# ChenAnno/FashionERN_AAAI2024

Hardware: AMD Instinct MI355X
Metric: composed queries/sec (higher is better)
Workload: dtype f32; 1 GPU; FashionIQ ViT-B/16 composed queries: 64-query batch per GPU vs 46k-image fused gallery (BASELINE.json configs[1]); clip=ViT-B-16, query_batch_per_gpu=64, gallery_rows=46000, gallery_dtype=f32, feature_dim=512, top_k=50, batches_in_flight=4, hw_queues=4, parallelism=dp1 queries

## Files before the change

### fashionern_aaai2024_amd/_lib.py

```python
from __future__ import annotations

import ctypes as C
import os

from . import build as _build

c_void_p, c_int, c_i64, c_float = C.c_void_p, C.c_int, C.c_int64, C.c_float

os.environ.setdefault("GPU_MAX_HW_QUEUES", "8")


class ClipConfigC(C.Structure):
    _fields_ = [(n, c_int) for n in (
        "embed_dim", "image_size", "patch_size", "v_width", "v_layers", "v_heads", "v_mlp",
        "context_length", "vocab_size", "t_width", "t_heads", "t_layers", "t_mlp", "v_arch")] + [
        ("r_layers", c_int * 4), ("r_width", c_int), ("r_heads", c_int)]


class ProfStats(C.Structure):
    _fields_ = [("gemm_ms", C.c_double), ("gemm_flops", C.c_double), ("gemm_launches", c_i64),
                ("attn_ms", C.c_double), ("attn_flops", C.c_double), ("attn_launches", c_i64),
                ("topk_ms", C.c_double), ("topk_launches", c_i64),
                ("sweep_ms", C.c_double), ("sweep_bytes", C.c_double), ("sweep_launches", c_i64),
                ("gemm_fp8_ms", C.c_double), ("gemm_fp8_flops", C.c_double), ("gemm_fp8_launches", c_i64),
# ... 73 lines not shown
    "fern_set_precision": (c_int, [c_void_p, c_int]),
    "fern_get_precision": (c_int, [c_void_p]),
    "fern_gemm_bf16": (c_int, [c_void_p, c_void_p, c_i64, c_void_p, c_i64, c_void_p, c_void_p, c_void_p, c_i64,
                               c_int, c_int, c_int, c_int, c_int, c_void_p]),
    "fern_quantize_rows_fp8": (c_int, [c_void_p, c_void_p, c_int, c_i64, c_void_p, c_i64, c_void_p, c_i64, c_int, c_void_p]),
    "fern_gemm_fp8": (c_int, [c_void_p, c_void_p, c_i64, c_void_p, c_void_p, c_i64, c_void_p, c_void_p, c_void_p, c_void_p, c_i64,
                              c_int, c_int, c_int, c_int, c_int, c_void_p]),
    "fern_quantize_mx8": (c_int, [c_void_p, c_void_p, c_int, c_i64, c_void_p, c_i64, c_void_p, c_i64, c_i64, c_int, c_void_p]),
    "fern_gemm_mx8": (c_int, [c_void_p, c_void_p, c_i64, c_void_p, c_i64, c_void_p, c_i64, c_void_p, c_i64, c_void_p, c_void_p, c_void_p, c_i64,
                              c_int, c_int, c_int, c_int, c_int, c_void_p]),
    "fern_gemm_mx8_quant": (c_int, [c_void_p, c_void_p, c_i64, c_void_p, c_i64, c_void_p, c_i64, c_void_p, c_i64, c_void_p, c_void_p, c_i64,
                                    c_void_p, c_i64, c_int, c_int, c_int, c_int, c_void_p]),
    "fern_layernorm": (c_int, [c_void_p, c_void_p, c_void_p, c_void_p, c_void_p, c_void_p, c_i64, c_int, c_float, c_void_p]),
    "fern_attention": (c_int, [c_void_p, c_void_p, c_i64, c_void_p, c_i64, c_void_p, c_i64, c_void_p, c_i64,
                               c_int, c_int, c_int, c_int, c_int, c_int, c_float, c_void_p]),
    "fern_attention_bf16": (c_int, [c_void_p, c_void_p, c_i64, c_void_p, c_i64, c_void_p, c_i64, c_void_p, c_i64,
                                    c_int, c_int, c_int, c_int, c_int, c_int, c_float, c_void_p]),
    "fern_layernorm_q": (c_int, [c_void_p, c_void_p, c_int, c_i64, c_void_p, c_void_p, c_int, c_void_p, c_i64, c_void_p, c_i64, c_i64,
                                 c_int, c_float, c_void_p]),
    "fern_attention_mx8": (c_int, [c_void_p, c_void_p, c_i64, c_void_p, c_i64, c_void_p, c_i64, c_void_p, c_i64, c_void_p, c_i64,
                                   c_int, c_int, c_int, c_int, c_int, c_int, c_float, c_void_p]),
    "fern_im2col_q": (c_int, [c_void_p, c_void_p, c_int, c_int, c_int, c_int, c_void_p, c_void_p, c_i64, c_void_p]),
    "fern_prof_enable": (c_int, [c_void_p, c_int]),
    "fern_prof_collect": (c_int, [c_void_p, C.POINTER(ProfStats)]),
    "fern_tuner_export": (c_i64, [C.c_char_p, c_i64]),
    "fern_tuner_import": (c_int, [C.c_char_p]),
    "fern_tuner_set_concurrency": (c_int, [c_int]),
    "fern_tuner_force_config": (c_int, [C.c_char_p, c_int]),
    "fern_ws_generation": (C.c_uint64, [c_void_p]),
}
# ... 34 lines not shown
```

### fashionern_aaai2024_amd/csrc/api_blocks.hip

```cpp
#include "ctx.h"

using namespace fern;
using namespace fern::api;

extern "C" int fern_resample_u8_horizontal(fern_ctx* c, const uint8_t* src, int64_t src_ld, int x0, int y0, int rows, uint8_t* dst, int ow,
                                           const int32_t* bounds, const int32_t* coeffs, int ksize, void* stream) {
    if (!c || !src || !dst || !bounds || !coeffs || rows < 0 || ow < 0 || ksize < 1) return fail(FERN_ERR_ARG, "fern_resample_u8_horizontal: bad argument");
    HIP_TRY(hipSetDevice(c->device));
    HIP_TRY(launch_resample_h(src, src_ld, x0, y0, rows, dst, ow, bounds, coeffs, ksize, (hipStream_t)stream));
    return FERN_OK;
}
extern "C" int fern_resample_u8_vertical(fern_ctx* c, const uint8_t* src, int64_t src_ld, int x0, int y0, int cols, uint8_t* dst, int oh,
                                         const int32_t* bounds, const int32_t* coeffs, int ksize, void* stream) {
    if (!c || !src || !dst || !bounds || !coeffs || cols < 0 || oh < 0 || ksize < 1) return fail(FERN_ERR_ARG, "fern_resample_u8_vertical: bad argument");
    HIP_TRY(hipSetDevice(c->device));
    HIP_TRY(launch_resample_v(src, src_ld, x0, y0, cols, dst, oh, bounds, coeffs, ksize, (hipStream_t)stream));
    return FERN_OK;
}
extern "C" int fern_u8_to_normalized_chw(fern_ctx* c, const uint8_t* src, int64_t src_ld, int x0, int y0, int64_t src_image_stride, float* dst,
                                         int n, int oh, int ow, const float* host_mean, const float* host_std, void* stream) {
    if (!c || !src || !dst || !host_mean || !host_std || n < 0 || oh < 0 || ow < 0) return fail(FERN_ERR_ARG, "fern_u8_to_normalized_chw: bad argument");
    HIP_TRY(hipSetDevice(c->device));
    HIP_TRY(launch_u8_to_chw(src, src_ld, x0, y0, dst, n, src_image_stride, oh, ow, host_mean, host_std, (hipStream_t)stream));
    return FERN_OK;
// ... 142 lines not shown
                              int64_t ldo, int batch, int heads, int head_dim, int s_q, int s_k, int causal, float scale, void* stream) {
    FERN_TRY(attn_begin(c, "fern_attention", q, k, v, out, ldq, ldk, ldv, ldo, heads, head_dim));
    AttnParams a{q, k, v, out, (long)ldq, (long)ldk, (long)ldv, (long)ldo, batch, heads, head_dim, s_q, s_k, causal, scale};
    return run_attention(c, a, (hipStream_t)stream);
}

extern "C" int fern_attention_bf16(fern_ctx* c, const uint16_t* q, int64_t ldq, const uint16_t* k, int64_t ldk, const uint16_t* v, int64_t ldv,
                                   uint16_t* out, int64_t ldo, int batch, int heads, int head_dim, int s_q, int s_k, int causal, float scale,
                                   void* stream) {
    FERN_TRY(attn_begin(c, "fern_attention_bf16", q, k, v, out, ldq, ldk, ldv, ldo, heads, head_dim));
    return run_attention(c, attn_desc_b(q, ldq, k, ldk, v, ldv, out, ldo, batch, heads, head_dim, s_q, s_k, causal, scale), (hipStream_t)stream);
}

static bool misaligned16(const void* p) { return (reinterpret_cast<uintptr_t>(p) & 15) != 0; }

extern "C" int fern_layernorm_q(fern_ctx* c, const void* x, int x_is_bf16, int64_t ldx, const float* gamma, const float* beta, int out_form,
                                void* y, int64_t ldy, void* scales, int64_t scale_rows, int64_t rows, int d, float eps, void* stream) {
    if (!c) return fail(FERN_ERR_ARG, "fern_layernorm_q: ctx is NULL");
    if (rows < 0 || (out_form != FERN_QFORM_BF16 && out_form != FERN_QFORM_FP8 && out_form != FERN_QFORM_MX8))
        return fail(FERN_ERR_ARG, "fern_layernorm_q: bad argument");
    if (rows == 0) return FERN_OK;
    if (!x || !gamma || !beta || !y || (out_form != FERN_QFORM_BF16 && !scales)) return fail(FERN_ERR_ARG, "fern_layernorm_q: NULL argument");
    if (d <= 0 || d % 4 || d > 1280 || ldx < d || ldy < d || ldx % 4 || ldy % 4)
        return fail(FERN_ERR_ARG, "fern_layernorm_q: need d % 4 == 0, d <= 1280, ld % 4 == 0, ld >= d");
    if (misaligned16(x) || misaligned16(gamma) || misaligned16(beta) || misaligned16(y) || (scales && misaligned16(scales)))
        return fail(FERN_ERR_ARG, "fern_layernorm_q: pointers must be 16-byte aligned");
    if (out_form == FERN_QFORM_MX8 && (d % 128 || scale_rows < rows))
        return fail(FERN_ERR_ARG, "fern_layernorm_q: the MX form needs d % 128 == 0 and scale_rows >= rows");
    if (out_form != FERN_QFORM_MX8 && x_is_bf16) return fail(FERN_ERR_ARG, "fern_layernorm_q: bf16 rows are read by the MX form only");
    HIP_TRY(hipSetDevice(c->device));
// ... 55 lines not shown
```

### fashionern_aaai2024_amd/csrc/api_ctx.hip

```cpp
#include <cstdio>
#include <cstdlib>
#include <cstring>
#include "ctx.h"

using namespace fern;
using namespace fern::api;

static thread_local std::string g_last_error;
int fern::api::fail(int code, const std::string& msg) {
    g_last_error = msg;
    return code;
}
extern "C" int fern_abi_version(void) { return FERN_ABI_VERSION; }
extern "C" const char* fern_last_error(void) { return g_last_error.c_str(); }

namespace fern {
thread_local LaunchTimer* g_launch_timer = nullptr;
hipEvent_t launch_timer_event() {
    LaunchTimer* t = g_launch_timer;
    hipEvent_t e = nullptr;
    if (t && t->pool && !t->pool->empty()) { e = t->pool->back(); t->pool->pop_back(); }
    else (void)hipEventCreate(&e);
    return e;
}
// ... 277 lines not shown
    const hipError_t le = launch_gemm_mxbf_pair(p1, p2, s);
    HIP_TRY_PROF(le, c, slot);
    if (slot >= 0) {
        c->recs[slot].dispatches = gemm_last_dispatches();
        c->recs[slot].extra_flops = 2.0 * p2.M * (double)p2.N * p2.K;
    }
    return prof_close(c, slot, s);
}
int fern::api::run_attention(fern_ctx* c, const AttnParams& a, hipStream_t s) {
    int slot;
    FERN_TRY(prof_open(c, PROF_ATTN, 4.0 * a.batch * a.heads * (double)a.s_q * a.s_k * a.hd, s, &slot, a.batch * a.heads, a.s_q, a.hd, a.causal));
    const hipError_t le = launch_attention(a, s);
    HIP_TRY_PROF(le, c, slot);
    return prof_close(c, slot, s);
}

extern "C" int fern_set_precision(fern_ctx* c, int precision) {
    if (!c) return fail(FERN_ERR_ARG, "fern_set_precision: ctx is NULL");
    if (precision != FERN_PREC_FP32 && precision != FERN_PREC_BF16 && precision != FERN_PREC_FP8 && precision != FERN_PREC_MX8 &&
        precision != FERN_PREC_F32X3 && precision != FERN_PREC_MX8_MLP && precision != FERN_PREC_MX8_IMG)
        return fail(FERN_ERR_ARG, "fern_set_precision: unknown precision");
    const bool split = precision == FERN_PREC_F32X3;
    if (split) precision = FERN_PREC_FP32;
    auto every_layer_has = [&](const unsigned char* LinearW::*copy) {
        for (const auto* blocks : {&c->clip.vblocks, &c->clip.tblocks})
            for (const auto& b : *blocks)
                if (!(b.qkv.*copy) || !(b.out.*copy) || !(b.fc.*copy) || !(b.proj.*copy)) return false;
        return true;
    };
    if ((precision == FERN_PREC_MX8 || precision == FERN_PREC_MX8_MLP || precision == FERN_PREC_MX8_IMG) && c->clip.ready && !every_layer_has(&LinearW::wm))
// ... 49 lines not shown
```

### fashionern_aaai2024_amd/csrc/api_towers.hip

```cpp
#include <cmath>
#include "ctx.h"

using namespace fern;
using namespace fern::api;

enum Form { F32, BF16, FP8, MX };

struct Tower {
    const ClipBlockW* blocks;
    int batch, S, width, heads, mlp, causal;
    Form attn, mlpf;
    bool bf16_stream;
    float *X, *XN, *QKV, *ATT, *H;
    unsigned short* Xb;

    long R() const { return (long)batch * S; }
    void* stream() const { return Xb ? (void*)Xb : (void*)X; }
    unsigned short* XNb() const { return reinterpret_cast<unsigned short*>(XN); }
    unsigned short* QKVb() const { return reinterpret_cast<unsigned short*>(QKV); }
    unsigned short* ATTb() const { return reinterpret_cast<unsigned short*>(ATT); }
    unsigned short* Hb() const { return reinterpret_cast<unsigned short*>(H); }
    unsigned char* XN8() const { return reinterpret_cast<unsigned char*>(XN); }
    float* SA() const { return XN + ((size_t)R() * width / 4 + 63) / 64 * 64; }
    unsigned char* SM() const { return reinterpret_cast<unsigned char*>(SA()); }
// ... 129 lines not shown
    FERN_TRY(run_gemm_form(c, T.mlpf, p, s));
    FERN_TRY(prep_proj(c, T, Bk, s, &p));
    return run_gemm_form(c, T.mlpf, p, s);
}

static int clip_block_cls_only(fern_ctx* c, const Tower& V, const ClipBlockW& Bk, float* CLS , float* T0 ,
                               float* T1 , float* H , hipStream_t s) {
    const int batch = V.batch, S = V.S, width = V.width, heads = V.heads, hd = width / heads;
    const float* X = V.X;
    const unsigned short* Xb = V.Xb;
    float* QKV = V.QKV;
    LinearW kv{Bk.qkv.w + (size_t)width * width, Bk.qkv.b + width, 2 * width, width, Bk.qkv.wb + (size_t)width * width,
               Bk.qkv.w8 ? Bk.qkv.w8 + (size_t)width * width : nullptr, Bk.qkv.sw ? Bk.qkv.sw + width : nullptr,
               Bk.qkv.wm ? Bk.qkv.wm + (size_t)width * width : nullptr, Bk.qkv.swm ? Bk.qkv.swm + (size_t)width * 4 : nullptr, Bk.qkv.swm_rows};
    const Form f = c->precision == FERN_PREC_MX8_IMG ? BF16 : V.attn;
    GemmParams pk;
    FERN_TRY(ln_gemm(V, f, Bk.ln1, kv, QKV + width, 3 * width, EPI_BIAS, false, s, &pk));
    FERN_TRY(run_gemm_form(c, f, pk, s));
    if (f == F32) {
        HIP_TRY(launch_gather_rows(V.XN, width, T0, width, batch, width, 1, S, 0, nullptr, s));
    } else {
        if (Xb) HIP_TRY(launch_gather_rows_bf16(Xb, width, T1, width, batch, width, S, s));
        else HIP_TRY(launch_gather_rows(X, width, T1, width, batch, width, 1, S, 0, nullptr, s));
        HIP_TRY(launch_layernorm(T1, nullptr, Bk.ln1.g, Bk.ln1.b, T0, batch, width, width, width, 1e-5f, s));
    }
    LinearW qw{Bk.qkv.w, Bk.qkv.b, width, width};
    FERN_TRY(run_gemm(c, gemm_desc(T0, width, qw, T1, width, batch, EPI_BIAS), s));
    AttnParams a{T1, QKV + width, QKV + 2 * width, T0, (long)width, 3L * width, 3L * width, (long)width,
                 batch, heads, hd, 1, S, 0, 1.0f / std::sqrt((float)hd)};
    FERN_TRY(run_attention(c, a, s));
    if (Xb) HIP_TRY(launch_gather_rows_bf16(Xb, width, CLS, width, batch, width, S, s));
    else HIP_TRY(launch_gather_rows(X, width, CLS, width, batch, width, 1, S, 0, nullptr, s));
    GemmParams po = gemm_desc(T0, width, Bk.out, CLS, width, batch, EPI_BIAS_RESIDUAL);
    po.R = CLS;
    FERN_TRY(run_gemm(c, po, s));
    HIP_TRY(launch_layernorm(CLS, nullptr, Bk.ln2.g, Bk.ln2.b, T0, batch, width, width, width, 1e-5f, s));
    FERN_TRY(run_gemm(c, gemm_desc(T0, width, Bk.fc, H, Bk.fc.out, batch, clip_mlp_epi(c)), s));
    GemmParams p2 = gemm_desc(H, Bk.fc.out, Bk.proj, CLS, width, batch, EPI_BIAS_RESIDUAL);
    p2.R = CLS;
    const int ks = (Bk.fc.out >= 2048 && Bk.fc.out % 512 == 0 && (width & 3) == 0) ? Bk.fc.out / 512 : 1;
    if (ks > 1) {
        float* kpart;
        FERN_TRY(ws_get(c, (size_t)ks * batch * width, &kpart));
        p2.ksplit = ks; p2.kpart = kpart; p2.epi = EPI_BIAS; p2.R = nullptr;
        FERN_TRY(run_gemm(c, p2, s));
// ... 113 lines not shown
static int resnet_chunk(fern_ctx* c, const float* images, float* out, int b, hipStream_t s) {
    const ClipW& W = c->clip;
    const ResNetW& R = W.res;
    const fern_clip_config& cf = W.cfg;
    const int S = cf.image_size, s1 = S / 2, w = cf.r_width;
    size_t max_act = (size_t)b * s1 * s1 * std::max(R.stem_c, w);
    {
        int H = S / 4;
        for (const auto& B : R.blocks) {
            max_act = std::max(max_act, (size_t)b * H * H * std::max(B.cin, B.planes * 4));
            if (B.stride > 1) H /= 2;
        }
    }
    {
        const int hf = S / 32;
        max_act = std::max(max_act, (size_t)b * (hf * hf + 1) * 2 * (size_t)(w * 32));
    }
    float* buf[6];
    for (auto& p : buf) FERN_TRY(ws_get(c, max_act, &p));
    HIP_TRY(launch_stem_conv(images, R.stem1.w, R.stem1.b, buf[0], b, S, R.stem_c, s));
    FERN_TRY(conv3x3(c, buf[0], R.stem2, buf[1], b, s1, s1, R.stem_c, s));
    FERN_TRY(conv3x3(c, buf[1], R.stem3, buf[0], b, s1, s1, R.stem_c, s));
    HIP_TRY(launch_avgpool_nhwc(buf[0], buf[1], b, s1, s1, w, 2, s));
    float* X = buf[1];
    float* OUT = buf[0];
    int H = S / 4;
    for (const auto& B : R.blocks) {
        const int rows = b * H * H, Ho = H / B.stride, rows_o = b * Ho * Ho;
        float *T1 = buf[2], *T2 = buf[3], *TP = buf[4], *ID = buf[5];
        FERN_TRY(run_gemm(c, conv_desc(X, B.c1, T1, rows, EPI_BIAS_RELU), s));
        FERN_TRY(conv3x3(c, T1, B.c2, T2, b, H, H, B.planes, s));
// ... 5 lines not shown
            HIP_TRY(launch_avgpool_nhwc(X, TP, b, H, H, B.cin, B.stride, s));
            xin = TP;
        }
        const float* identity = X;
        if (B.has_down) {
            FERN_TRY(run_gemm(c, conv_desc(xin, B.down, ID, rows_o, EPI_BIAS), s));
            identity = ID;
        }
        GemmParams p3 = conv_desc(t2, B.c3, OUT, rows_o, EPI_BIAS_RESIDUAL_RELU);
        p3.R = identity;
        FERN_TRY(run_gemm(c, p3, s));
        std::swap(X, OUT);
        H = Ho;
    }
    const int HW = H * H, E = w * 32, heads = cf.r_heads, hd = E / heads;
    float *T = buf[2], *T0 = buf[3], *MEAN = buf[3] + (size_t)b * E, *KV = buf[4], *Q = buf[5], *ATT = buf[5] + (size_t)b * E;
    HIP_TRY(launch_attnpool_tokens(X, MEAN, R.pos, T, T0, b, HW, E, s));
    FERN_TRY(run_gemm(c, gemm_desc(T, E, R.kv, KV, 2 * E, b * (HW + 1), EPI_BIAS), s));
    FERN_TRY(run_gemm(c, gemm_desc(T0, E, R.q, Q, E, b, EPI_BIAS), s));
    AttnParams a{Q, KV, KV + E, ATT, (long)E, 2L * E, 2L * E, (long)E, b, heads, hd, 1, HW + 1, 0, 1.0f / std::sqrt((float)hd)};
    FERN_TRY(run_attention(c, a, s));
    return run_gemm(c, gemm_desc(ATT, E, R.cproj, out, cf.embed_dim, b, EPI_BIAS), s);
}

extern "C" int fern_vit_encode_image(fern_ctx* c, const float* images, float* out, int b, void* stream) {
    if (!c) return fail(FERN_ERR_ARG, "fern_vit_encode_image: ctx is NULL");
    if (!c->clip.ready || (c->clip.cfg.v_arch == 0 && c->clip.cfg.v_layers <= 0))
        return fail(FERN_ERR_STATE, "fern_vit_encode_image: image tower not finalised (fern_finalize_clip)");
    FERN_TRY(check_fresh(c, "fern_vit_encode_image"));
    if (b < 0 || (b && (!images || !out))) return fail(FERN_ERR_ARG, "fern_vit_encode_image: bad argument");
    HIP_TRY(hipSetDevice(c->device));
    hipStream_t s = (hipStream_t)stream;
    const fern_clip_config& cf = c->clip.cfg;
    const long img_sz = 3L * cf.image_size * cf.image_size;
    const bool resnet = cf.v_arch == 1;
    const int CH = resnet ? 128 : vit_chunk_images(cf);
// ... 123 lines not shown
```

### fashionern_aaai2024_amd/csrc/attn.hip

```cpp
#include "kernels.h"

#include <cstdlib>

namespace fern {

typedef float f32x16 __attribute__((ext_vector_type(16)));
typedef float f32x4 __attribute__((ext_vector_type(4)));
typedef short bf16x8 __attribute__((ext_vector_type(8)));
typedef short s16x4 __attribute__((ext_vector_type(4)));
typedef unsigned u32x4_t __attribute__((ext_vector_type(4)));

extern __shared__ __attribute__((aligned(16))) char attn_smem[];

struct LanePos { int l31, lh, tr_off; };
__device__ __forceinline__ LanePos lane_pos() {
    const int lane = threadIdx.x & 63, lh = lane >> 5;
    return {lane & 31, lh, ((lane & 15) >> 2) * 64 + (((lane >> 4) & 1) * 16 + (lane & 3) * 4) * 2 + lh * 4 * 64};
}

template <int HDP_>
struct F32Form {
    static constexpr int HDP = HDP_;
    static constexpr bool BF16 = false;
    static constexpr int KS = HDP + 4;
// ... 464 lines not shown
        for (int u = 0; u < UNR; ++u) {
            const int j = j0 + 4 * u;
            vv[u] = vb[(long)(j < p.s_k ? j : p.s_k - 1) * p.ldv];
        }
#pragma unroll
        for (int u = 0; u < UNR; ++u) {
            const int j = j0 + 4 * u;
            acc = __builtin_fmaf(j < p.s_k ? sc[j] : 0.0f, vv[u], acc);
        }
    }
    red[wave][lane] = acc;
    __syncthreads();
    if (wave == 0 && lane < hd)
        p.out[(long)b * p.ldo + (long)h * hd + lane] = (((red[0][lane] + red[1][lane]) + red[2][lane]) + red[3][lane]) * (1.0f / sum);
}
hipError_t launch_attention(const AttnParams& p, hipStream_t s) {
    if (p.batch <= 0 || p.heads <= 0 || p.s_q <= 0 || p.s_k <= 0 || p.s_k > ATTN_MAX_KEYS) return hipErrorInvalidValue;
    if (p.causal && p.s_q != p.s_k) return hipErrorInvalidValue;
    if (p.qb || p.kb || p.vb) {
        if (!p.qb || !p.kb || !p.vb || (!p.out_b && !p.out_q8) || (p.out_q8 && (!p.out_scales || (p.hd & 31))) || (p.hd & 7) || (p.ldq & 7) || (p.ldk & 7) || (p.ldv & 7) || (p.ldo & 3)) return hipErrorInvalidValue;
        return launch_hd<Bf16Form>(p, s);
    }
    if (p.out_b || p.out_q8) return hipErrorInvalidValue;
    if ((p.hd & 3) || (p.ldq & 3) || (p.ldk & 3) || (p.ldv & 3) || (p.ldo & 3)) return hipErrorInvalidValue;
    if (p.s_q == 1 && !p.causal && p.hd <= 64 && p.s_k <= SQ1_MAX_KEYS) {
        FERN_LAUNCH(attn_f32_single_query_kernel<25>, dim3(p.batch * p.heads), dim3(256), 0, s, p);
        return hipGetLastError();
    }
    return launch_hd<F32Form>(p, s);
}
// ... 3 lines not shown
```

### fashionern_aaai2024_amd/csrc/ctx.h

```cpp
#pragma once
#include <hip/hip_runtime.h>
#include <algorithm>
#include <cstdint>
#include <map>
#include <string>
#include <vector>
#include "../../include/fern.h"
#include "kernels.h"

namespace fern::api {
int fail(int code, const std::string& msg);

#define HIP_TRY(expr)                                                                                   \
    do {                                                                                                \
        hipError_t e_ = (expr);                                                                         \
        if (e_ != hipSuccess)                                                                           \
            return ::fern::api::fail(e_ == hipErrorInvalidValue ? FERN_ERR_ARG : FERN_ERR_HIP,          \
                        std::string(#expr) + ": " + hipGetErrorString(e_) + " (" __FILE__ ":" + std::to_string(__LINE__) + ")"); \
    } while (0)
#define FERN_TRY(expr)              \
    do {                            \
        int r_ = (expr);            \
        if (r_ != FERN_OK) return r_; \
    } while (0)
// ... 122 lines not shown
    bool on = false, done = false;
    int sweep_lo = 0, sweep_hi = 0;
    double sweep_bytes = 0;
    StageTimer(fern_ctx* ctx, hipStream_t s);
    void sweep_begin() { if (on) sweep_lo = (int)c->timer.events.size() / 2; }
    void sweep_end(double bytes) { if (on) { sweep_hi = (int)c->timer.events.size() / 2; sweep_bytes += bytes; } }
    void commit(int m, int n, int k);
    ~StageTimer();
};

int run_gemm(fern_ctx* c, const GemmParams& p, hipStream_t s, int kind = PROF_GEMM, double work = -1.0);
int run_gemm_pair(fern_ctx* c, const GemmParams& p1, const GemmParams& p2, hipStream_t s);
int run_gemm_b(fern_ctx* c, const GemmParams& p, hipStream_t s);
int run_gemm_b_pair(fern_ctx* c, const GemmParams& p1, const GemmParams& p2, hipStream_t s);
int run_attention(fern_ctx* c, const AttnParams& a, hipStream_t s);
GemmParams gemm_desc(const float* A, long lda, const LinearW& L, float* C, long ldc, int M, int epi);
GemmParams gemm_desc_b(const unsigned short* A, long lda, const LinearW& L, void* C, long ldc, int M, int epi, bool out_bf16);
GemmParams gemm_desc_f8(const unsigned char* A8, const float* sa, long lda, const LinearW& L, void* C, long ldc, int M, int epi, bool out_bf16);
GemmParams gemm_desc_mx(const unsigned char* A8, const unsigned char* sa, long srows, long lda, const LinearW& L, void* C, long ldc, int M, int epi, bool out_bf16);
int clip_mlp_epi(const fern_ctx* c);

int check_fresh(fern_ctx* c, const char* fn);
int check_token_flag(fern_ctx* c, const char* fn);
int check_live_flags(fern_ctx* c, const char* fn);

}
```

### fashionern_aaai2024_amd/csrc/kernels.h

```cpp
#pragma once
#include <hip/hip_runtime.h>
#include <stdint.h>

#include <string>

#ifdef __HIPCC__
#include <hip/hip_ext.h>
#endif
#include <vector>

namespace fern {

struct LaunchTimer {
    std::vector<hipEvent_t> events;
    std::vector<hipEvent_t>* pool;
};
extern thread_local LaunchTimer* g_launch_timer;
struct LaunchTimerPause {
    LaunchTimer* saved;
    LaunchTimerPause() : saved(g_launch_timer) { g_launch_timer = nullptr; }
    ~LaunchTimerPause() { g_launch_timer = saved; }
};
hipEvent_t launch_timer_event();
#ifdef __HIPCC__
// ... 201 lines not shown
struct AttnParams {
    const float* q; const float* k; const float* v; float* out;
    long ldq, ldk, ldv, ldo;
    int batch, heads, hd, s_q, s_k, causal;
    float scale;
    unsigned short* out_b;
    const unsigned short* qb;
    const unsigned short* kb;
    const unsigned short* vb;
    unsigned char* out_q8;
    unsigned char* out_scales;
    long out_srows;
};
constexpr int ATTN_MAX_KEYS = 4096;
hipError_t launch_attention(const AttnParams& p, hipStream_t s);

hipError_t launch_layernorm(const float* x, const float* res, const float* gamma, const float* beta, float* y,
                            long rows, int d, long ldx, long ldy, float eps, hipStream_t s);
hipError_t launch_layernorm_bf16(const float* x, const float* gamma, const float* beta, unsigned short* y, long rows, int d, long ldx,
                                 long ldy, float eps, hipStream_t s);
hipError_t launch_layernorm_fp8(const float* x, const float* gamma, const float* beta, unsigned char* y, float* scale, long rows, int d,
                                long ldx, long ldy, float eps, hipStream_t s);
hipError_t launch_quantize_rows_fp8(const unsigned short* x_bf16, const float* x_f32, long ldx, unsigned char* y, long ldy, float* scale,
                                    long rows, int d, hipStream_t s);
hipError_t launch_layernorm_mx8(const float* x, const float* gamma, const float* beta, unsigned char* y, unsigned char* scales, long srows,
                                long rows, int d, long ldx, long ldy, float eps, hipStream_t s, const unsigned short* x_bf16 = nullptr );
hipError_t launch_quantize_mx8(const unsigned short* x_bf16, const float* x_f32, long ldx, unsigned char* y, long ldy, unsigned char* scales,
                               long srows, long rows, int d, hipStream_t s);
hipError_t launch_im2col_bf16(const float* images, unsigned short* y, int b, int img, int patch, int grid, hipStream_t s);
hipError_t launch_patch_rows_f32(const float* images, float* y, int b, int img, int patch, int grid, int kp, hipStream_t s);
// ... 108 lines not shown
```

### fashionern_aaai2024_amd/engine.py

```python
from __future__ import annotations

import ctypes as C
import sys
from typing import Dict, Mapping, Optional

import numpy as np
import torch

from . import _lib
from .synth import ClipConfig

COMBINER_TARGET, COMBINER_DVR_GLOBAL, COMBINER_DVR_LOCAL, COMBINER_DVR_FINAL = 0, 1, 2, 3
SR_TARGET, SR_DVR = 0, 1
EPI_BIAS, EPI_BIAS_GELU, EPI_BIAS_RELU, EPI_BIAS_RESIDUAL = 0, 1, 2, 3
EPI_BIAS_QUICKGELU = 4
ACT_GELU, ACT_QUICK_GELU = 0, 1
PART_DVR, PART_TARGET_SR, PART_TARGET_COMBINER, PART_ALL = 1, 2, 4, 7
PREC_FP32, PREC_BF16, PREC_FP8, PREC_MX8, PREC_F32X3, PREC_MX8_MLP, PREC_MX8_IMG = 0, 1, 2, 3, 4, 5, 6
QFORM_BF16, QFORM_FP8, QFORM_MX8 = 0, 1, 2
_PREC_NAMES = {"fp32": PREC_FP32, "bf16": PREC_BF16, "fp8": PREC_FP8, "mx8": PREC_MX8, "f32x3": PREC_F32X3, "mx8mlp": PREC_MX8_MLP, "mx8img": PREC_MX8_IMG}
PATCH_NUM = 13


def _ptr(t: Optional[torch.Tensor]):
# ... 810 lines not shown
        _lib.check(self.lib.fern_layernorm(self._h, _ptr(x), _ptr(residual), _ptr(gamma), _ptr(beta), _ptr(out), rows, d,
                                           float(eps), _stream()), "fern_layernorm")
        return out

    def attention(self, q, k, v, heads: int, causal=False, scale=None) -> torch.Tensor:
        q, k, v = self._f32(q), self._f32(k), self._f32(v)
        b, sq, w = q.shape
        sk = k.shape[1]
        hd = w // heads
        out = torch.empty_like(q)
        sc = float(scale) if scale is not None else hd ** -0.5
        _lib.check(self.lib.fern_attention(self._h, _ptr(q), w, _ptr(k), w, _ptr(v), w, _ptr(out), w, b, heads, hd, sq, sk,
                                           int(bool(causal)), sc, _stream()), "fern_attention")
        return out

    def attention_bf16(self, q, k, v, heads: int, causal=False, scale=None) -> torch.Tensor:
        def b16(x):
            if x.dtype != torch.bfloat16:
                x3 = self._f32(x)
                return self.to_bf16(x3.reshape(-1, x3.shape[-1])).reshape(x3.shape)
            return x.to(self.device).contiguous()
        q, k, v = b16(q), b16(k), b16(v)
        b, sq, w = q.shape
        sk = k.shape[1]
        hd = w // heads
        out = torch.empty_like(q)
        sc = float(scale) if scale is not None else hd ** -0.5
        _lib.check(self.lib.fern_attention_bf16(self._h, _ptr(q), w, _ptr(k), w, _ptr(v), w, _ptr(out), w, b, heads, hd, sq, sk,
                                                int(bool(causal)), sc, _stream()), "fern_attention_bf16")
        return out
# ... 86 lines not shown
```

### include/fern.h

```cpp
#ifndef FERN_H
#define FERN_H

#include <stddef.h>
#include <stdint.h>

#ifdef __cplusplus
extern "C" {
#endif

#define FERN_ABI_VERSION 3

#if defined(__GNUC__)
#define FERN_API __attribute__((visibility("default")))
#else
#define FERN_API
#endif

typedef struct fern_ctx fern_ctx;

typedef enum {
    FERN_OK = 0,
    FERN_ERR_ARG = -1,
    FERN_ERR_HIP = -2,
    FERN_ERR_STATE = -3,
// ... 235 lines not shown
                  const float* scale_w, const float* bias, const float* residual, void* C, int64_t ldc, int M, int N, int K,
                  int epilogue, int out_bf16, void* stream);
FERN_API int fern_quantize_mx8(fern_ctx* ctx, const void* x, int x_is_bf16, int64_t ldx, uint8_t* y, int64_t ldy, uint8_t* scales,
                      int64_t scale_rows, int64_t rows, int d, void* stream);
FERN_API int fern_gemm_mx8(fern_ctx* ctx, const uint8_t* A, int64_t lda, const uint8_t* scales_a, int64_t scale_rows_a, const uint8_t* W,
                  int64_t ldw, const uint8_t* scales_w, int64_t scale_rows_w, const float* bias, const float* residual, void* C,
                  int64_t ldc, int M, int N, int K, int epilogue, int out_bf16, void* stream);
FERN_API int fern_gemm_mx8_quant(fern_ctx* ctx, const uint8_t* A, int64_t lda, const uint8_t* scales_a, int64_t scale_rows_a, const uint8_t* W,
                        int64_t ldw, const uint8_t* scales_w, int64_t scale_rows_w, const float* bias, uint8_t* C8, int64_t ldc,
                        uint8_t* scales_c, int64_t scale_rows_c, int M, int N, int K, int epilogue, void* stream);
FERN_API int fern_layernorm(fern_ctx* ctx, const float* x, const float* residual, const float* gamma,
                   const float* beta, float* y, int64_t rows, int d, float eps, void* stream);
FERN_API int fern_attention(fern_ctx* ctx, const float* q, int64_t ldq, const float* k, int64_t ldk, const float* v,
                   int64_t ldv, float* out, int64_t ldo, int batch, int heads, int head_dim, int s_q,
                   int s_k, int causal, float scale, void* stream);
FERN_API int fern_attention_bf16(fern_ctx* ctx, const uint16_t* q, int64_t ldq, const uint16_t* k, int64_t ldk, const uint16_t* v,
                        int64_t ldv, uint16_t* out, int64_t ldo, int batch, int heads, int head_dim, int s_q, int s_k,
                        int causal, float scale, void* stream);
FERN_API int fern_layernorm_q(fern_ctx* ctx, const void* x, int x_is_bf16, int64_t ldx, const float* gamma, const float* beta, int out_form,
                     void* y, int64_t ldy, void* scales, int64_t scale_rows, int64_t rows, int d, float eps, void* stream);
FERN_API int fern_attention_mx8(fern_ctx* ctx, const uint16_t* q, int64_t ldq, const uint16_t* k, int64_t ldk, const uint16_t* v,
                       int64_t ldv, uint8_t* out, int64_t ldo, uint8_t* scales, int64_t scale_rows, int batch, int heads,
                       int head_dim, int s_q, int s_k, int causal, float scale, void* stream);
FERN_API int fern_im2col_q(fern_ctx* ctx, const float* images, int b, int img, int patch, int out_form, void* y, void* scales,
                  int64_t scale_rows, void* stream);

FERN_API int64_t fern_tuner_export(char* buf, int64_t cap);
FERN_API int fern_tuner_import(const char* text);
FERN_API int fern_tuner_set_concurrency(int lanes);
FERN_API int fern_tuner_force_config(const char* family, int cfg);
// ... 11 lines not shown
```

Before: 2955 queries/sec.

## Fold K/V projections into single-query pooled attention to skip full KV GEMM

For single-query attention pooling (the ViT last-block CLS path in F32 and the ResNet attnpool), the kernel stops projecting every token to K and V. It folds the query through Wk into a per-head query in token space, scores the raw tokens, takes the softmax-weighted token sum, and only then applies Wv plus bias per head. This removes the large K/V GEMM over all tokens and its activation buffer, which is why the workspace sizing shrinks. The cost is three new custom kernels plus extra per-head work, and the K bias is dropped from the scores on the assumption that it is constant across keys and cancels in the softmax.

```diff
diff --git a/fashionern_aaai2024_amd/_lib.py b/fashionern_aaai2024_amd/_lib.py
--- a/fashionern_aaai2024_amd/_lib.py
+++ b/fashionern_aaai2024_amd/_lib.py
@@ -111,6 +111,8 @@
     "fern_layernorm": (c_int, [c_void_p, c_void_p, c_void_p, c_void_p, c_void_p, c_void_p, c_i64, c_int, c_float, c_void_p]),
     "fern_attention": (c_int, [c_void_p, c_void_p, c_i64, c_void_p, c_i64, c_void_p, c_i64, c_void_p, c_i64,
                                c_int, c_int, c_int, c_int, c_int, c_int, c_float, c_void_p]),
+    "fern_pooled_attention": (c_int, [c_void_p, c_void_p, c_i64, c_void_p, c_i64, c_i64, c_void_p, c_void_p, c_void_p, c_void_p, c_i64,
+                                      c_int, c_int, c_int, c_int, c_void_p]),
     "fern_attention_bf16": (c_int, [c_void_p, c_void_p, c_i64, c_void_p, c_i64, c_void_p, c_i64, c_void_p, c_i64,
                                     c_int, c_int, c_int, c_int, c_int, c_int, c_float, c_void_p]),
     "fern_layernorm_q": (c_int, [c_void_p, c_void_p, c_int, c_i64, c_void_p, c_void_p, c_int, c_void_p, c_i64, c_void_p, c_i64, c_i64,
diff --git a/fashionern_aaai2024_amd/csrc/api_blocks.hip b/fashionern_aaai2024_amd/csrc/api_blocks.hip
--- a/fashionern_aaai2024_amd/csrc/api_blocks.hip
+++ b/fashionern_aaai2024_amd/csrc/api_blocks.hip
@@ -180,6 +180,28 @@
 
 static bool misaligned16(const void* p) { return (reinterpret_cast<uintptr_t>(p) & 15) != 0; }
 
+extern "C" int fern_pooled_attention(fern_ctx* c, const float* q, int64_t ldq, const float* tokens, int64_t ldt, int64_t image_stride,
+                                     const float* wk, const float* wv, const float* bv, float* out, int64_t ldo, int batch, int heads,
+                                     int head_dim, int s, void* stream) {
+    if (!c) return fail(FERN_ERR_ARG, "fern_pooled_attention: ctx is NULL");
+    if (!q || !tokens || !wk || !wv || !bv || !out) return fail(FERN_ERR_ARG, "fern_pooled_attention: NULL argument");
+    const int64_t E = (int64_t)heads * head_dim;
+    if (batch <= 0 || heads <= 0 || head_dim <= 0 || head_dim % 4 || head_dim > 128 || E > POOLED_MAX_E || s <= 0 || s > POOLED_MAX_KEYS)
+        return fail(FERN_ERR_ARG, "fern_pooled_attention: need head_dim % 4 == 0, head_dim <= 128, heads * head_dim <= " +
+                                      std::to_string(POOLED_MAX_E) + ", 1 <= s <= " + std::to_string(POOLED_MAX_KEYS));
+    if (ldq < E || ldt < E || ldo < E || ldq % 4 || ldt % 4 || ldo % 4 || image_stride % 4 || image_stride < (int64_t)(s - 1) * ldt + E)
+        return fail(FERN_ERR_ARG, "fern_pooled_attention: need ldq, ldt, ldo >= heads * head_dim, strides % 4 == 0, image_stride >= (s - 1) * ldt + heads * head_dim");
+    if (misaligned16(q) || misaligned16(tokens) || misaligned16(wk) || misaligned16(wv) || misaligned16(bv) || misaligned16(out))
+        return fail(FERN_ERR_ARG, "fern_pooled_attention: pointers must be 16-byte aligned");
+    HIP_TRY(hipSetDevice(c->device));
+    const hipStream_t st = (hipStream_t)stream;
+    FERN_TRY(ws_begin(c, st));
+    PooledAttnParams a{q, (long)ldq, tokens, (long)ldt, (long)image_stride, wk, wv, (long)E, bv, out, (long)ldo, nullptr, nullptr,
+                       batch, heads, head_dim, s, 1.0f / std::sqrt((float)head_dim)};
+    return run_pooled_attention(c, a, st);
+}
+
+
 extern "C" int fern_layernorm_q(fern_ctx* c, const void* x, int x_is_bf16, int64_t ldx, const float* gamma, const float* beta, int out_form,
                                 void* y, int64_t ldy, void* scales, int64_t scale_rows, int64_t rows, int d, float eps, void* stream) {
     if (!c) return fail(FERN_ERR_ARG, "fern_layernorm_q: ctx is NULL");
diff --git a/fashionern_aaai2024_amd/csrc/api_ctx.hip b/fashionern_aaai2024_amd/csrc/api_ctx.hip
--- a/fashionern_aaai2024_amd/csrc/api_ctx.hip
+++ b/fashionern_aaai2024_amd/csrc/api_ctx.hip
@@ -315,6 +315,18 @@
     HIP_TRY_PROF(le, c, slot);
     return prof_close(c, slot, s);
 }
+int fern::api::run_pooled_attention(fern_ctx* c, const PooledAttnParams& p, hipStream_t s) {
+    PooledAttnParams a = p;
+    const double E = (double)a.heads * a.hd;
+    if (a.batch <= 0 || a.heads <= 0 || a.hd <= 0) return fail(FERN_ERR_ARG, "pooled attention: bad shape");
+    FERN_TRY(ws_get(c, (size_t)a.batch * a.heads * (size_t)E, &a.qt));
+    FERN_TRY(ws_get(c, (size_t)a.batch * a.heads * (size_t)E, &a.u));
+    int slot;
+    FERN_TRY(prof_open(c, PROF_ATTN, 4.0 * a.batch * E * E + 4.0 * a.batch * a.heads * (double)a.S * E, s, &slot, a.batch * a.heads, 1, (int)E, 2));
+    const hipError_t le = launch_pooled_attention(a, s);
+    HIP_TRY_PROF(le, c, slot);
+    return prof_close(c, slot, s);
+}
 
 extern "C" int fern_set_precision(fern_ctx* c, int precision) {
     if (!c) return fail(FERN_ERR_ARG, "fern_set_precision: ctx is NULL");
diff --git a/fashionern_aaai2024_amd/csrc/api_towers.hip b/fashionern_aaai2024_amd/csrc/api_towers.hip
--- a/fashionern_aaai2024_amd/csrc/api_towers.hip
+++ b/fashionern_aaai2024_amd/csrc/api_towers.hip
@@ -167,9 +167,14 @@
                Bk.qkv.w8 ? Bk.qkv.w8 + (size_t)width * width : nullptr, Bk.qkv.sw ? Bk.qkv.sw + width : nullptr,
                Bk.qkv.wm ? Bk.qkv.wm + (size_t)width * width : nullptr, Bk.qkv.swm ? Bk.qkv.swm + (size_t)width * 4 : nullptr, Bk.qkv.swm_rows};
     const Form f = c->precision == FERN_PREC_MX8_IMG ? BF16 : V.attn;
-    GemmParams pk;
-    FERN_TRY(ln_gemm(V, f, Bk.ln1, kv, QKV + width, 3 * width, EPI_BIAS, false, s, &pk));
-    FERN_TRY(run_gemm_form(c, f, pk, s));
+    const bool pooled = f == F32 && S <= POOLED_MAX_KEYS && width <= POOLED_MAX_E && hd <= 128;
+    if (pooled) {
+        HIP_TRY(launch_layernorm(X, nullptr, Bk.ln1.g, Bk.ln1.b, V.XN, V.R(), width, width, width, 1e-5f, s));
+    } else {
+        GemmParams pk;
+        FERN_TRY(ln_gemm(V, f, Bk.ln1, kv, QKV + width, 3 * width, EPI_BIAS, false, s, &pk));
+        FERN_TRY(run_gemm_form(c, f, pk, s));
+    }
     if (f == F32) {
         HIP_TRY(launch_gather_rows(V.XN, width, T0, width, batch, width, 1, S, 0, nullptr, s));
     } else {
@@ -179,9 +184,15 @@
     }
     LinearW qw{Bk.qkv.w, Bk.qkv.b, width, width};
     FERN_TRY(run_gemm(c, gemm_desc(T0, width, qw, T1, width, batch, EPI_BIAS), s));
-    AttnParams a{T1, QKV + width, QKV + 2 * width, T0, (long)width, 3L * width, 3L * width, (long)width,
-                 batch, heads, hd, 1, S, 0, 1.0f / std::sqrt((float)hd)};
-    FERN_TRY(run_attention(c, a, s));
+    if (pooled) {
+        PooledAttnParams a{T1, (long)width, V.XN, (long)width, (long)S * width, kv.w, kv.w + (size_t)width * width, (long)width, kv.b + width,
+                           T0, (long)width, nullptr, nullptr, batch, heads, hd, S, 1.0f / std::sqrt((float)hd)};
+        FERN_TRY(run_pooled_attention(c, a, s));
+    } else {
+        AttnParams a{T1, QKV + width, QKV + 2 * width, T0, (long)width, 3L * width, 3L * width, (long)width,
+                     batch, heads, hd, 1, S, 0, 1.0f / std::sqrt((float)hd)};
+        FERN_TRY(run_attention(c, a, s));
+    }
     if (Xb) HIP_TRY(launch_gather_rows_bf16(Xb, width, CLS, width, batch, width, S, s));
     else HIP_TRY(launch_gather_rows(X, width, CLS, width, batch, width, 1, S, 0, nullptr, s));
     GemmParams po = gemm_desc(T0, width, Bk.out, CLS, width, batch, EPI_BIAS_RESIDUAL);
@@ -325,7 +336,7 @@
     }
     {
         const int hf = S / 32;
-        max_act = std::max(max_act, (size_t)b * (hf * hf + 1) * 2 * (size_t)(w * 32));
+        max_act = std::max(max_act, (size_t)b * (hf * hf + 1) * (size_t)(w * 32));
     }
     float* buf[6];
     for (auto& p : buf) FERN_TRY(ws_get(c, max_act, &p));
@@ -361,12 +372,12 @@
         H = Ho;
     }
     const int HW = H * H, E = w * 32, heads = cf.r_heads, hd = E / heads;
-    float *T = buf[2], *T0 = buf[3], *MEAN = buf[3] + (size_t)b * E, *KV = buf[4], *Q = buf[5], *ATT = buf[5] + (size_t)b * E;
+    float *T = buf[2], *T0 = buf[3], *MEAN = buf[3] + (size_t)b * E, *Q = buf[5], *ATT = buf[5] + (size_t)b * E;
     HIP_TRY(launch_attnpool_tokens(X, MEAN, R.pos, T, T0, b, HW, E, s));
-    FERN_TRY(run_gemm(c, gemm_desc(T, E, R.kv, KV, 2 * E, b * (HW + 1), EPI_BIAS), s));
     FERN_TRY(run_gemm(c, gemm_desc(T0, E, R.q, Q, E, b, EPI_BIAS), s));
-    AttnParams a{Q, KV, KV + E, ATT, (long)E, 2L * E, 2L * E, (long)E, b, heads, hd, 1, HW + 1, 0, 1.0f / std::sqrt((float)hd)};
-    FERN_TRY(run_attention(c, a, s));
+    PooledAttnParams a{Q, (long)E, T, (long)E, (long)(HW + 1) * E, R.kv.w, R.kv.w + (size_t)E * E, (long)E, R.kv.b + E,
+                       ATT, (long)E, nullptr, nullptr, b, heads, hd, HW + 1, 1.0f / std::sqrt((float)hd)};
+    FERN_TRY(run_pooled_attention(c, a, s));
     return run_gemm(c, gemm_desc(ATT, E, R.cproj, out, cf.embed_dim, b, EPI_BIAS), s);
 }
 
diff --git a/fashionern_aaai2024_amd/csrc/attn.hip b/fashionern_aaai2024_amd/csrc/attn.hip
--- a/fashionern_aaai2024_amd/csrc/attn.hip
+++ b/fashionern_aaai2024_amd/csrc/attn.hip
@@ -502,6 +502,210 @@
     if (wave == 0 && lane < hd)
         p.out[(long)b * p.ldo + (long)h * hd + lane] = (((red[0][lane] + red[1][lane]) + red[2][lane]) + red[3][lane]) * (1.0f / sum);
 }
+
+static_assert(POOLED_MAX_KEYS == SQ1_MAX_KEYS, "the pooled form takes the key counts of the single-query kernel");
+
+template <int N, int M>
+__device__ __forceinline__ void lane_fold(float* v, int lane) {
+    if constexpr (M >= 1) {
+        if constexpr (N > 1) {
+            constexpr int H = N / 2;
+            const bool up = (lane & M) != 0;
+#pragma unroll
+            for (int i = 0; i < H; ++i) {
+                const float send = up ? v[i] : v[i + H];
+                const float keep = up ? v[i + H] : v[i];
+                v[i] = keep + __shfl_xor(send, M);
+            }
+            lane_fold<H, M / 2>(v, lane);
+        } else {
+            v[0] += __shfl_xor(v[0], M);
+            lane_fold<1, M / 2>(v, lane);
+        }
+    }
+}
+__device__ __forceinline__ float dot4_acc(const float4& a, const float4& b, float acc) {
+    acc = __builtin_fmaf(a.x, b.x, acc);
+    acc = __builtin_fmaf(a.y, b.y, acc);
+    acc = __builtin_fmaf(a.z, b.z, acc);
+    return __builtin_fmaf(a.w, b.w, acc);
+}
+__device__ __forceinline__ void axpy4(float a, const float4& x, float4& y) {
+    y.x = __builtin_fmaf(a, x.x, y.x);
+    y.y = __builtin_fmaf(a, x.y, y.y);
+    y.z = __builtin_fmaf(a, x.z, y.z);
+    y.w = __builtin_fmaf(a, x.w, y.w);
+}
+
+constexpr int POOL_BT = 16;
+constexpr int POOL_HG = 4;
+constexpr int POOL_NW = 8;
+
+__global__ __launch_bounds__(64) void pooled_fold_kernel(PooledAttnParams p) {
+    __shared__ float qs[POOL_BT * 128];
+    const int lane = threadIdx.x, b0 = blockIdx.x * POOL_BT, h = blockIdx.z, hd = p.hd, E = p.heads * hd;
+    for (int idx = lane; idx < POOL_BT * hd; idx += 64) {
+        const int i = idx / hd, d = idx - i * hd;
+        const int b = b0 + i < p.batch ? b0 + i : p.batch - 1;
+        qs[idx] = p.q[(long)b * p.ldq + (long)h * hd + d];
+    }
+    __syncthreads();
+    const int col = blockIdx.y * 256 + lane * 4;
+    if (col >= E) return;
+    float4 acc[POOL_BT];
+#pragma unroll
+    for (int i = 0; i < POOL_BT; ++i) acc[i] = float4{0.f, 0.f, 0.f, 0.f};
+    const float* w = p.wk + (long)h * hd * p.ldw + col;
+#pragma unroll 4
+    for (int d = 0; d < hd; ++d) {
+        const float4 w4 = *reinterpret_cast<const float4*>(w + (long)d * p.ldw);
+#pragma unroll
+        for (int i = 0; i < POOL_BT; ++i) axpy4(qs[i * hd + d], w4, acc[i]);
+    }
+#pragma unroll
+    for (int i = 0; i < POOL_BT; ++i) {
+        if (b0 + i >= p.batch) break;
+        const float4 r{acc[i].x * p.scale, acc[i].y * p.scale, acc[i].z * p.scale, acc[i].w * p.scale};
+        *reinterpret_cast<float4*>(p.qt + ((long)(b0 + i) * p.heads + h) * E + col) = r;
+    }
+}
+
+__global__ __launch_bounds__(POOL_NW * 64) void pooled_tokens_kernel(PooledAttnParams p) {
+    extern __shared__ __align__(16) float pool_lds[];
+    const int tid = threadIdx.x, lane = tid & 63, wave = tid >> 6;
+    const int b = blockIdx.x, h0 = blockIdx.y * POOL_HG, S = p.S, E = p.heads * p.hd;
+    float* qs = pool_lds;
+    float* red = qs + (size_t)POOL_HG * E;
+    float* sc = red + POOL_NW * POOL_HG * 256;
+    float* sinv = sc + (size_t)POOL_HG * S;
+    for (int idx = tid * 4; idx < POOL_HG * E; idx += POOL_NW * 256) {
+        const int g = idx / E, e = idx - g * E;
+        const int h = h0 + g < p.heads ? h0 + g : p.heads - 1;
+        *reinterpret_cast<float4*>(qs + idx) = *reinterpret_cast<const float4*>(p.qt + ((long)b * p.heads + h) * E + e);
+    }
+    __syncthreads();
+    const float* tb = p.tok + (long)b * p.img_stride;
+    for (int j0 = wave * 4; j0 < S; j0 += POOL_NW * 4) {
+        float acc[4 * POOL_HG];
+#pragma unroll
+        for (int i = 0; i < 4 * POOL_HG; ++i) acc[i] = 0.f;
+        const float* tr[4];
+#pragma unroll
+        for (int u = 0; u < 4; ++u) tr[u] = tb + (long)(j0 + u < S ? j0 + u : S - 1) * p.ldt;
+        for (int c = lane * 4; c < E; c += 256) {
+            float4 t4[4];
+#pragma unroll
+            for (int u = 0; u < 4; ++u) t4[u] = *reinterpret_cast<const float4*>(tr[u] + c);
+#pragma unroll
+            for (int g = 0; g < POOL_HG; ++g) {
+                const float4 q4 = *reinterpret_cast<const float4*>(qs + (size_t)g * E + c);
+#pragma unroll
+                for (int u = 0; u < 4; ++u) acc[u * POOL_HG + g] = dot4_acc(q4, t4[u], acc[u * POOL_HG + g]);
+            }
+        }
+        lane_fold<4 * POOL_HG, 32>(acc, lane);
+        const int idx = (lane >> 2) & 15, j = j0 + idx / POOL_HG;
+        if ((lane & 3) == 0 && j < S) sc[(idx % POOL_HG) * S + j] = acc[0];
+    }
+    __syncthreads();
+    if (wave < POOL_HG) {
+        float* s = sc + (size_t)wave * S;
+        float mx = -INFINITY;
+        for (int j = lane; j < S; j += 64) mx = fmaxf(mx, s[j]);
+#pragma unroll
+        for (int m = 32; m >= 1; m >>= 1) mx = fmaxf(mx, __shfl_xor(mx, m));
+        float sum = 0.f;
+        for (int j = lane; j < S; j += 64) {
+            const float e = expf(s[j] - mx);
+            s[j] = e;
+            sum += e;
+        }
+#pragma unroll
+        for (int m = 32; m >= 1; m >>= 1) sum += __shfl_xor(sum, m);
+        if (lane == 0) sinv[wave] = 1.0f / sum;
+    }
+    __syncthreads();
+    for (int c0 = 0; c0 < E; c0 += 256) {
+        const int c = c0 + lane * 4;
+        float4 acc[POOL_HG];
+#pragma unroll
+        for (int g = 0; g < POOL_HG; ++g) acc[g] = float4{0.f, 0.f, 0.f, 0.f};
+        if (c < E) {
+#pragma unroll 4
+            for (int j = wave; j < S; j += POOL_NW) {
+                const float4 t4 = *reinterpret_cast<const float4*>(tb + (long)j * p.ldt + c);
+#pragma unroll
+                for (int g = 0; g < POOL_HG; ++g) axpy4(sc[g * S + j], t4, acc[g]);
+            }
+        }
+#pragma unroll
+        for (int g = 0; g < POOL_HG; ++g) *reinterpret_cast<float4*>(red + ((wave * POOL_HG + g) * 256 + lane * 4)) = acc[g];
+        __syncthreads();
+        for (int o = tid; o < POOL_HG * 256; o += POOL_NW * 64) {
+            const int g = o >> 8, cl = o & 255;
+            if (c0 + cl < E && h0 + g < p.heads) {
+                float sum = red[g * 256 + cl];
+#pragma unroll
+                for (int w = 1; w < POOL_NW; ++w) sum += red[(w * POOL_HG + g) * 256 + cl];
+                p.u[((long)b * p.heads + h0 + g) * E + c0 + cl] = sum * sinv[g];
+            }
+        }
+        __syncthreads();
+    }
+}
+
+__global__ __launch_bounds__(256) void pooled_vproj_kernel(PooledAttnParams p) {
+    const int lane = threadIdx.x & 63, wave = threadIdx.x >> 6;
+    const int b0 = blockIdx.x * POOL_BT, d0 = blockIdx.y * 16 + wave * 4, h = blockIdx.z, hd = p.hd, E = p.heads * hd;
+    if (d0 >= hd) return;
+    float acc[4 * POOL_BT];
+#pragma unroll
+    for (int i = 0; i < 4 * POOL_BT; ++i) acc[i] = 0.f;
+    const float* wr[4];
+#pragma unroll
+    for (int r = 0; r < 4; ++r) wr[r] = p.wv + ((long)h * hd + (d0 + r < hd ? d0 + r : hd - 1)) * p.ldw;
+    const float* ur[POOL_BT];
+#pragma unroll
+    for (int i = 0; i < POOL_BT; ++i) ur[i] = p.u + ((long)(b0 + i < p.batch ? b0 + i : p.batch - 1) * p.heads + h) * E;
+    for (int c = lane * 4; c < E; c += 256) {
+        float4 w4[4];
+#pragma unroll
+        for (int r = 0; r < 4; ++r) w4[r] = *reinterpret_cast<const float4*>(wr[r] + c);
+#pragma unroll
+        for (int i = 0; i < POOL_BT; ++i) {
+            const float4 u4 = *reinterpret_cast<const float4*>(ur[i] + c);
+#pragma unroll
+            for (int r = 0; r < 4; ++r) acc[r * POOL_BT + i] = dot4_acc(w4[r], u4, acc[r * POOL_BT + i]);
+        }
+    }
+    lane_fold<4 * POOL_BT, 32>(acc, lane);
+    const int d = d0 + lane / POOL_BT, b = b0 + lane % POOL_BT;
+    if (d < hd && b < p.batch) p.out[(long)b * p.ldo + (long)h * hd + d] = p.bv[h * hd + d] + acc[0];
+}
+
+hipError_t launch_pooled_attention(const PooledAttnParams& p, hipStream_t s) {
+    const long E = (long)p.heads * p.hd;
+    if (p.batch <= 0 || p.heads <= 0 || p.hd <= 0 || (p.hd & 3) || p.hd > 128 || E > POOLED_MAX_E || p.S <= 0 || p.S > POOLED_MAX_KEYS)
+        return hipErrorInvalidValue;
+    if ((p.ldq & 3) || (p.ldt & 3) || (p.img_stride & 3) || (p.ldw & 3) || (p.ldo & 3) || p.ldq < E || p.ldt < E || p.ldw < E || p.ldo < E)
+        return hipErrorInvalidValue;
+    for (const void* ptr : {(const void*)p.q, (const void*)p.tok, (const void*)p.wk, (const void*)p.wv, (const void*)p.bv, (const void*)p.out,
+                            (const void*)p.qt, (const void*)p.u})
+        if (!ptr || (reinterpret_cast<uintptr_t>(ptr) & 15)) return hipErrorInvalidValue;
+    const unsigned bt = (p.batch + POOL_BT - 1) / POOL_BT, ec = (unsigned)((E + 255) / 256);
+    const size_t lds = sizeof(float) * ((size_t)POOL_HG * E + POOL_NW * POOL_HG * 256 + (size_t)POOL_HG * p.S + POOL_HG);
+    static size_t lds_allowed = 48 * 1024;
+    if (lds > lds_allowed) {
+        hipError_t e = hipFuncSetAttribute(reinterpret_cast<const void*>(pooled_tokens_kernel), hipFuncAttributeMaxDynamicSharedMemorySize, (int)lds);
+        if (e != hipSuccess) return e;
+        lds_allowed = lds;
+    }
+    FERN_LAUNCH(pooled_fold_kernel, dim3(bt, ec, p.heads), dim3(64), 0, s, p);
+    FERN_LAUNCH(pooled_tokens_kernel, dim3(p.batch, (p.heads + POOL_HG - 1) / POOL_HG), dim3(POOL_NW * 64), lds, s, p);
+    FERN_LAUNCH(pooled_vproj_kernel, dim3(bt, (p.hd + 15) / 16, p.heads), dim3(256), 0, s, p);
+    return hipGetLastError();
+}
+
 hipError_t launch_attention(const AttnParams& p, hipStream_t s) {
     if (p.batch <= 0 || p.heads <= 0 || p.s_q <= 0 || p.s_k <= 0 || p.s_k > ATTN_MAX_KEYS) return hipErrorInvalidValue;
     if (p.causal && p.s_q != p.s_k) return hipErrorInvalidValue;
diff --git a/fashionern_aaai2024_amd/csrc/ctx.h b/fashionern_aaai2024_amd/csrc/ctx.h
--- a/fashionern_aaai2024_amd/csrc/ctx.h
+++ b/fashionern_aaai2024_amd/csrc/ctx.h
@@ -160,6 +160,7 @@
 int run_gemm_b(fern_ctx* c, const GemmParams& p, hipStream_t s);
 int run_gemm_b_pair(fern_ctx* c, const GemmParams& p1, const GemmParams& p2, hipStream_t s);
 int run_attention(fern_ctx* c, const AttnParams& a, hipStream_t s);
+int run_pooled_attention(fern_ctx* c, const PooledAttnParams& p, hipStream_t s);
 GemmParams gemm_desc(const float* A, long lda, const LinearW& L, float* C, long ldc, int M, int epi);
 GemmParams gemm_desc_b(const unsigned short* A, long lda, const LinearW& L, void* C, long ldc, int M, int epi, bool out_bf16);
 GemmParams gemm_desc_f8(const unsigned char* A8, const float* sa, long lda, const LinearW& L, void* C, long ldc, int M, int epi, bool out_bf16);
diff --git a/fashionern_aaai2024_amd/csrc/kernels.h b/fashionern_aaai2024_amd/csrc/kernels.h
--- a/fashionern_aaai2024_amd/csrc/kernels.h
+++ b/fashionern_aaai2024_amd/csrc/kernels.h
@@ -239,6 +239,18 @@
 };
 constexpr int ATTN_MAX_KEYS = 4096;
 hipError_t launch_attention(const AttnParams& p, hipStream_t s);
+struct PooledAttnParams {
+    const float* q; long ldq;
+    const float* tok; long ldt, img_stride;
+    const float* wk; const float* wv; long ldw;
+    const float* bv;
+    float* out; long ldo;
+    float* qt; float* u;
+    int batch, heads, hd, S;
+    float scale;
+};
+constexpr int POOLED_MAX_KEYS = 1024, POOLED_MAX_E = 4096;
+hipError_t launch_pooled_attention(const PooledAttnParams& p, hipStream_t s);
 
 hipError_t launch_layernorm(const float* x, const float* res, const float* gamma, const float* beta, float* y,
                             long rows, int d, long ldx, long ldy, float eps, hipStream_t s);
diff --git a/fashionern_aaai2024_amd/engine.py b/fashionern_aaai2024_amd/engine.py
--- a/fashionern_aaai2024_amd/engine.py
+++ b/fashionern_aaai2024_amd/engine.py
@@ -848,6 +848,15 @@
                                            int(bool(causal)), sc, _stream()), "fern_attention")
         return out
 
+    def pooled_attention(self, q, tokens, wk, wv, bv, heads: int) -> torch.Tensor:
+        q, tokens = self._f32(q), self._f32(tokens)
+        b, s, e = tokens.shape
+        wk, wv, bv = self._f32(wk, (e, e)), self._f32(wv, (e, e)), self._f32(bv, (e,))
+        out = torch.empty_like(q)
+        _lib.check(self.lib.fern_pooled_attention(self._h, _ptr(q), e, _ptr(tokens), e, s * e, _ptr(wk), _ptr(wv), _ptr(bv), _ptr(out), e,
+                                                  b, heads, e // heads, s, _stream()), "fern_pooled_attention")
+        return out
+
     def attention_bf16(self, q, k, v, heads: int, causal=False, scale=None) -> torch.Tensor:
         def b16(x):
             if x.dtype != torch.bfloat16:
diff --git a/include/fern.h b/include/fern.h
--- a/include/fern.h
+++ b/include/fern.h
@@ -273,6 +273,9 @@
 FERN_API int fern_attention(fern_ctx* ctx, const float* q, int64_t ldq, const float* k, int64_t ldk, const float* v,
                    int64_t ldv, float* out, int64_t ldo, int batch, int heads, int head_dim, int s_q,
                    int s_k, int causal, float scale, void* stream);
+FERN_API int fern_pooled_attention(fern_ctx* ctx, const float* q, int64_t ldq, const float* tokens, int64_t ldt, int64_t image_stride,
+                   const float* wk, const float* wv, const float* bv, float* out, int64_t ldo, int batch, int heads,
+                   int head_dim, int s, void* stream);
 FERN_API int fern_attention_bf16(fern_ctx* ctx, const uint16_t* q, int64_t ldq, const uint16_t* k, int64_t ldk, const uint16_t* v,
                         int64_t ldv, uint16_t* out, int64_t ldo, int batch, int heads, int head_dim, int s_q, int s_k,
                         int causal, float scale, void* stream);
```

New measurement: 2985 queries/sec (median of 6 runs). 1.01x the previous value.
